# mightypirate1/DRL-Tetris

Hardware: AMD Instinct MI355X
Metric: env-steps/sec at 64k parallel 20x10 boards (higher is better)
Workload: dtype u32

## Files before the change

drl-tetris_amd/csrc/tetris_dev_rollout.h:

```cpp

constexpr int CHAIN_LANES = 64;
constexpr int CHAIN_STREAMS = 3;
template <int P, bool AFFINE, bool FUSED>
__device__ __forceinline__ void chain_body(const KArgs& a) {
    __shared__ __attribute__((aligned(16))) uint32_t s_shapes[SHAPE_WORDS];
    const int lane = threadIdx.x;
    if (a.steps < 0) { chain_census(a, lane == 0); return; }
    constexpr int CMEM = AFFINE ? MEM_AFFINE : MEM_AGENT;
    int wave = blockIdx.x;
    uint32_t xcc = 0;
    const auto report_xcc = [&]() { if (AFFINE && blockIdx.x == 0 && lane == 0) st_flag(a.status + F_XCC0 + (a.xcd_slot & 3u), 0x100u | xcc); };
    if (AFFINE) {
        asm volatile("s_getreg_b32 %0, hwreg(HW_REG_XCC_ID)" : "=s"(xcc));
        xcc &= 0xFu;
        if (xcc != ((a.xcd_base + blockIdx.x) & 7u)) {
            if (lane == 0) st_flag(a.status + F_PLACE, 1u);
            report_xcc();
            return;
        }
        wave = (int)((blockIdx.x & ~7u) | xcc);
        if (wave * CHAIN_LANES >= a.n) { report_xcc(); return; }
    }
    const int i = wave * CHAIN_LANES + lane;
    const bool active = lane < CHAIN_LANES && i < a.n;
    LaneCounters cnt = {0, 0, 0, 0};
    const uint32_t shape_word = d_shape_table.s[lane];
    Game<P> g;
    if (active) policy_draw(a, (uint32_t)i, a.first_step, g.draw0, g.draw1);
    const uint32_t d0 = g.draw0, d1 = g.draw1;
    int stride = a.n_stride;
    asm volatile("" : "+s"(stride));
    RowTable<NWORDS> rows = {};
    RowTable<NGWORDS> grows = {};
    if (!FUSED) {
        TE_UNROLL
        for (int w = 0; w < NWORDS; w++)
            if (P > 1 || (w < NWORDS_HOT && w != W_INCOMING && w != W_HOLE_DRAWS)) {
                uint32_t bytes = (uint32_t)(w * P) * (uint32_t)stride * 4u;
                asm volatile("" : "+s"(bytes));
                rows.bytes[w] = bytes;
            }
        TE_UNROLL
        for (int w = 0; w < NGWORDS; w++) {
            uint32_t bytes = (uint32_t)w * (uint32_t)stride * 4u;
// ... 4 lines not shown
    const uint32_t seen = chain_poll(a, (uint32_t)wave);
    if (seen == a.epoch - 1u) {
        Geo geo = geo_of(a);
        geo.stride = (size_t)stride;
        if (active) {
            if (FUSED) load_game<P>(geo, (size_t)i, g, false, P > 1, true, CMEM);
            else load_game_rows<P>(geo, (size_t)i, rows, grows, g, false, P > 1, true, CMEM);
            g.draw0 = d0; g.draw1 = d1;
        }
        s_shapes[lane] = shape_word;
        __builtin_amdgcn_wave_barrier();
        if (FUSED) {
            if (active) game_run<P, M_ROLLOUT, false, CMEM>(a, i, s_shapes, g, cnt);
        } else if (active) {
            const Ctx cx = make_ctx(a, s_shapes, false, P > 1);
            rollout_step<P>(cx, a, (size_t)i, a.first_step, g, cnt);
            store_game_rows<P>(geo, (size_t)i, rows, grows, g, false, P > 1, true, CMEM);
            report_status(a, g.status);
        }
        asm volatile("s_waitcnt vmcnt(0)" ::: "memory");
        if (lane == 0) {
            if (AFFINE) st_xcd(a.chain + (size_t)wave * CHAIN_STRIDE, a.epoch);
            else st_agent(a.chain + (size_t)wave * CHAIN_STRIDE, a.epoch);
        }
    } else if (!(seen & CHAIN_ABANDONED)) {
        chain_give_up(a, (uint32_t)wave, lane == 0);
    }
    report_xcc();
}
template <int P>
__global__ __launch_bounds__(64) void k_chain(KArgs a) { chain_body<P, false, false>(a); }
template <int P>
__global__ __launch_bounds__(64) void k_chain_affine(KArgs a) { chain_body<P, true, false>(a); }
template <int P>
__global__ __launch_bounds__(64) void k_chain_fused(KArgs a) { chain_body<P, false, true>(a); }
template <int P>
__global__ __launch_bounds__(64) void k_chain_fused_affine(KArgs a) { chain_body<P, true, true>(a); }
template __global__ void k_chain_affine<1>(KArgs);
// ... 45 lines not shown
    }
    if (active) {
        load_game_words<1>(gr, g, ROLL, MEM);
        load_player(br.s, br.o, br.ws, q, false, true, MEM);
        if (CHAIN) { g.draw0 = pd0; g.draw1 = pd1; }
        else if (ROLL) policy_draw(a, (uint32_t)gi, a.first_step, g.draw0, g.draw1);
        else { g.draw0 = a.rot[gi]; g.draw1 = (uint32_t)a.trans[gi] | ((a.player ? (uint32_t)a.player[gi] : 0u) << 8); }
    }
    s_shapes[lane] = shape_word;
    __builtin_amdgcn_wave_barrier();
    Ctx cx = make_ctx(a, s_shapes, false);
    uint32_t my_lines = 0, my_sent = 0;
    int done = 0, out_reward = 0, out_dead = 0;
    {
        int r = 0, t = 0, acting = 0;
        ResetPrefetch rpf;
        rpf.ok = 0; rpf.seed16 = 0; rpf.word = 0;
        uint32_t sent_start = 0;
        uint32_t wa = 0;
        uint32_t undo_pose = 0, undo_group = 0, undo_draws = 0, undo_cleared = 0;
        bool undo_ran = false;
        Player pre;
        if (active) {
            if (ROLL) {
                r = (int)(g.draw0 & 3u); t = (int)(g.draw1 % 10u); acting = (int)(a.first_step % 2ull);
            } else {
                r = (int)(g.draw0 & 3u); t = (int)(g.draw1 & 0xFFu); acting = (int)(g.draw1 >> 8);
            }
            if (ROLL || AUTO) prefetch_reset(cx, episode_seed(a.game_offset + (uint32_t)gi, g.episode + 1), rpf);
            prefetch_next(cx, q, g.seed16, g.status);
            sent_start = q.lines_sent;
            if (!g.round_over && !q.dead && acting == side) play_rt(cx, q, r, t);
            if (!CHAIN && side == 1) pre = q;
            undo_pose = pose_pack(q);
            undo_group = q.pgroup; undo_draws = q.piece_draws;
            undo_cleared = q.lines_cleared; undo_ran = !g.round_over && !q.dead;
            wa = split_settle(cx, g);
        }
        const uint32_t opp_a = __shfl_xor(wa, 32);
        uint32_t wb0 = 0, wb1 = 0;
        if (active) {
            if (side == 1 && (opp_a & XW_DIED)) {
                if (!CHAIN) {
                    q = pre;
// ... 20 lines not shown
        }
        const uint32_t x1 = __shfl_xor(wb1, 32);
        if (active) {
            const uint32_t opp_b = side == 0 ? x1 : x0;
            const int in = (side == 0 && !(opp_b & XW_DIED)) ? xw_sent(opp_b) : 0;
            g.flags = (uint32_t)side;
            done = split_finish(g, in, (opp_b & XW_DEAD_NOW) != 0, (opp_b & XW_ERR) != 0);
            out_reward = q.reward; out_dead = q.dead;
            if (ROLL) {
                g.steps++;
                if (!q.dead) my_lines += (unsigned)q.reward;
                my_sent += (q.lines_sent - sent_start) & 0xFFFFu;
            }
            if ((ROLL || AUTO) && done) {
                g.episode++;
                reset_split(cx, g, episode_seed(a.game_offset + (uint32_t)gi, g.episode));
            }
        }
    }
    const uint32_t opp_lines = __shfl_xor(my_lines, 32), opp_sent = __shfl_xor(my_sent, 32);
    if (active) {
        store_player(br.s, br.o, br.ws, q, false, true, MEM);
        if (!ROLL) {
            if (a.lines) a.lines[(size_t)side * a.n + gi] = (uint8_t)out_reward;
            if (a.dead) a.dead[(size_t)side * a.n + gi] = (uint8_t)out_dead;
        }
        const uint32_t st = g.status | __shfl_xor(g.status, 32);
        if (side == 0) {
            if (!ROLL && a.done) a.done[gi] = (uint8_t)done;
            g.flags = 0;
            g.add_lines = my_lines + opp_lines;
// ... 79 lines not shown
```

drl-tetris_amd/csrc/tetris_engine.h:

```cpp
#pragma once
#include "tetris_layout.h"
#include "tetris_tables.h"

#if defined(__clang__)
#define TE_UNROLL _Pragma("unroll")
#else
#define TE_UNROLL _Pragma("GCC unroll 8")
#endif

namespace te {

TE_HD int ctz32(uint32_t v) { return __builtin_ctz(v); }
TE_HD int clz32(uint32_t v) { return __builtin_clz(v); }
#if defined(__HIP_DEVICE_COMPILE__)
TE_HD uint32_t ld_stream(const uint32_t* p) { return __builtin_nontemporal_load(p); }
TE_HD void st_stream(uint32_t* p, uint32_t v) { __builtin_nontemporal_store(v, p); }
#else
TE_HD uint32_t ld_stream(const uint32_t* p) { return *p; }
TE_HD void st_stream(uint32_t* p, uint32_t v) { *p = v; }
#endif

#if defined(TE_PATH_COUNTERS) && !defined(__HIPCC__)
enum PathCounter { PC_KICK = 0, PC_KICK_2ND, PC_KICK_3RD, PC_KICK_FAILED, PC_KICK_DOWN, PC_DROP_EXACT, PC_RT_OFF_SPAWN,
                   PC_GARBAGE_ROW, PC_GARBAGE_LIFT2, PC_DEATH_GARBAGE, PC_DEATH_SPAWN, PC_TIMER_LOCK, PC_KEY_KICK, PC_KEY_KICK_FAILED,
// ... 43 lines not shown
struct RowStride { size_t ws; };
template <int N>
struct RowTable { uint32_t bytes[N]; };
TE_HD size_t row_bytes(const RowStride& r, int w) { return (size_t)w * r.ws * 4u; }
template <int N>
TE_HD size_t row_bytes(const RowTable<N>& r, int w) { return r.bytes[w]; }
#if defined(__HIP_DEVICE_COMPILE__)
TE_HD void add_word(uint32_t* p, uint32_t v) { (void)__hip_atomic_fetch_add(p, v, __ATOMIC_RELAXED, __HIP_MEMORY_SCOPE_AGENT); }
#else
TE_HD void add_word(uint32_t* p, uint32_t v) { *p += v; }
#endif
#if defined(__HIP_DEVICE_COMPILE__)
TE_HD uint32_t mul24(uint32_t a, uint32_t b) { return __umul24(a, b); }
#else
TE_HD uint32_t mul24(uint32_t a, uint32_t b) { return a * b; }
#endif
TE_HD int imin(int a, int b) { return a < b ? a : b; }
TE_HD int imax(int a, int b) { return a > b ? a : b; }
TE_HD uint32_t f2u(float f) { union { float f; uint32_t u; } v; v.f = f; return v.u; }
TE_HD float u2f(uint32_t u) { union { float f; uint32_t u; } v; v.u = u; return v.f; }

constexpr uint16_t SHAPE_ROWS[7][4] = {
    {0x2260, 0x0710, 0x3220, 0x4700}, {0x2230, 0x1700, 0x6220, 0x0740}, {0x2640, 0x0630, 0x1320, 0x6300},
    {0x2310, 0x3600, 0x4620, 0x0360}, {0x2222, 0x0f00, 0x4444, 0x00f0}, {0x0720, 0x2320, 0x2700, 0x2620},
    {0x0660, 0x0660, 0x0660, 0x0660},
};
TE_HD int spawn_rot(int kind) { return (int)((0x0977u >> (2 * (kind & 7))) & 3u); }
TE_HD int shape_value(int kind) { return (int)((0x06127534u >> (4 * (kind & 7))) & 15u); }

constexpr uint32_t make_shape(int kind, int rot) {
// ... 60 lines not shown
    int q_overflow;
    int32_t time_ms, drop_delay, drop_time, speedup_time, lock_time;
    int32_t combo_start, combo_time, min_remaining;
    uint32_t combo_remaining;
    float incoming;
    uint32_t piece_draws, hole_draws;
    uint32_t pgroup;
    uint32_t lines_sent, lines_cleared, lines_blocked, max_combo, lines_seen, garbage_cleared;
    int32_t qcount[FIFO_CAP];
    int32_t qdelay[FIFO_CAP];
    int q_loaded;
    Raw8 pf_raw;
    int pf_ok;
};

struct ResetPrefetch { uint32_t seed16; uint64_t word; int ok; };

template <int P>
struct Game {
    Player pl[P];
    uint32_t seed16;
    int round_over, last_winner;
    uint32_t flags;
    uint32_t episode;
    uint32_t steps;
    uint32_t add_lines, add_sent;
    uint32_t status;
    uint32_t draw0, draw1;
};

template <class ROWS>
// ... 249 lines not shown
        uint32_t above = (1u << r) - 1u;
        uint32_t keep = ~((above << 1) | 1u);
        if (cx.tint) {
            uint32_t garbage = 0;
            for (int c = 0; c < NCOL; c++) garbage |= q.col[c] & q.tint[0][c] & q.tint[1][c] & q.tint[2][c];
            if ((garbage >> r) & 1u) q.garbage_cleared = (q.garbage_cleared + 1u) & 0xFFFFu;
            for (int k = 0; k < 3; k++)
                for (int c = 0; c < NCOL; c++) q.tint[k][c] = (q.tint[k][c] & keep) | ((q.tint[k][c] & above) << 1);
        }
        for (int c = 0; c < NCOL; c++) q.col[c] = (q.col[c] & keep) | ((q.col[c] & above) << 1);
        cleared++;
    }
    return cleared;
}

TE_HD uint32_t table_byte(const Ctx& cx, uint32_t seed16, uint32_t draw, uint32_t& status) {
    if (draw + cx.margin >= cx.n_draws) {
        status |= ST_NEED_EXTEND;
        if (draw >= cx.n_draws) { status |= ST_STREAM_EXHAUSTED; draw = cx.n_draws - 1; }
    }
    uint32_t chunk = draw / (uint32_t)CHUNK;
    uint32_t r = draw - mul24(chunk, (uint32_t)CHUNK);
    return cx.table[mul24((chunk << 16) + seed16, (uint32_t)CHUNK) + r];
}

TE_HD Raw8 table_group_raw(const Ctx& cx, uint32_t seed16, uint32_t draw, uint32_t& status) {
    if (draw + 8u + cx.margin >= cx.n_draws) {
        status |= ST_NEED_EXTEND;
        if (draw + 8u > cx.n_draws) { status |= ST_STREAM_EXHAUSTED; draw = cx.n_draws - 8u; }
    }
    uint32_t chunk = draw / (uint32_t)CHUNK;
    uint32_t r = draw - mul24(chunk, (uint32_t)CHUNK);
    const uint8_t* p = cx.table + (mul24((chunk << 16) + seed16, (uint32_t)CHUNK) + r);
    Raw8 v;
#if defined(__HIP_DEVICE_COMPILE__)
    const uint2 w = *reinterpret_cast<const uint2*>(p);
    v.lo = w.x; v.hi = w.y;
#else
    v.lo = 0; v.hi = 0;
    for (int k = 0; k < 4; k++) { v.lo |= (uint32_t)p[k] << (8 * k); v.hi |= (uint32_t)p[4 + k] << (8 * k); }
#endif
    return v;
}
TE_HD uint32_t pack_group(Raw8 v) {
    const uint32_t a = v.lo & 0x0F0F0F0Fu, b = v.hi & 0x0F0F0F0Fu;
    uint32_t lo = (a | (a >> 4)) & 0x00FF00FFu; lo = (lo | (lo >> 8)) & 0x0000FFFFu;
    uint32_t hi = (b | (b >> 4)) & 0x00FF00FFu; hi = (hi | (hi >> 8)) & 0x0000FFFFu;
    return lo | (hi << 16);
// ... 79 lines not shown
TE_HD int combo_expire(const Ctx& cx, Player& q, int32_t t) {
    int32_t left = q.combo_start + q.combo_time - t;
    q.combo_remaining = left < 0 ? 0u : ((uint32_t)left & 0xFFFFu);
    if (t > q.combo_start + q.combo_time && q.combo_count != 0) {
        float duration = 1.f + (float)t / 60000.f * 0.1f;
        double v = cx.combo_pow[q.combo_count] * (double)duration;
        int lines = (int)((uint32_t)(int64_t)v & 0xFFFFu);
        q.combo_count = 0;
        q.line_count = 0;
        return lines;
    }
    return 0;
}


TE_HD bool spawn_next(const Ctx& cx, Player& q, uint32_t seed16, uint32_t& status) {
    q.kind = q.next;
    q.rot = spawn_rot(q.kind);
    q.x = (NCOL - 4) / 2;
    q.y = 0;
    if (q.piece_draws + cx.margin >= cx.n_draws) {
        status |= ST_NEED_EXTEND;
        if (q.piece_draws >= cx.n_draws) status |= ST_STREAM_EXHAUSTED;
    }
    q.next = (int)((q.pgroup >> (4u * (q.piece_draws & 7u))) & 7u);
    q.piece_draws++;
    if ((q.piece_draws & 7u) == 0u) {
        q.pgroup = pack_group(q.pf_ok ? q.pf_raw : table_group_raw(cx, seed16, q.piece_draws, status));
        q.pf_ok = 0;
    }
    uint32_t shape = shape_of(cx, q.kind, q.rot);
    if (!fits_spawn_col(cx, q, shape, 0)) { stamp(cx, q, shape); TE_COUNT(PC_DEATH_SPAWN); return true; }
    return false;
}

TE_HD int score_clears(const Ctx& cx, Player& q, int cleared) {
    q.lines_cleared = (q.lines_cleared + (uint32_t)cleared) & 0xFFFFu;
    if (cleared == 0) { q.combo_time -= 200; return 0; }
    int amount = cx.queue ? q_block(q, cleared - 1, q.time_ms, true) : cleared - 1;
    q.lines_sent = (q.lines_sent + (uint32_t)amount) & 0xFFFFu;
    combo_gain(q, q.time_ms, cleared);
    return amount;
}

TE_HD void lock_piece(const Ctx& cx, Player& q) {
    uint32_t shape = shape_of(cx, q.kind, q.rot);
    q.y += drop_distance(cx, q, shape);
    stamp(cx, q, shape);
    q.drop_time = q.time_ms;
    q.lock_armed = 0;
}

TE_HD int settle(const Ctx& cx, Player& q, uint32_t seed16, uint32_t& status) {
    int sent = score_clears(cx, q, clear_rows(cx, q));
    if (spawn_next(cx, q, seed16, status)) return -1;
    return sent;
}

TE_HD bool soft_drop(const Ctx& cx, Player& q) {
    const uint32_t shape = shape_of(cx, q.kind, q.rot);
    if (q.x == (NCOL - 4) / 2 ? fits_spawn_col(cx, q, shape, q.y + 1) : fits_at(cx, q, shape, q.x, q.y + 1)) {
        q.y++;
        q.drop_time = q.time_ms;
        q.lock_armed = 0;
        return true;
    }
    if (!q.lock_armed) q.lock_time = q.time_ms + 400;
    q.lock_armed = 1;
    return false;
}

TE_HD bool gravity_due(Player& q, int32_t t) {
    if (t - q.speedup_time > 3000) {
        if (q.drop_delay > 200) q.drop_delay -= 10;
        else if (q.drop_delay > 100) q.drop_delay -= 5;
        else if (q.drop_delay > 50) q.drop_delay -= 2;
        else if (q.drop_delay > 10) q.drop_delay -= 1;
        q.speedup_time = t;
    }
    if (t - q.drop_time > q.drop_delay) { q.drop_time = t; return true; }
    return false;
}

TE_HD bool push_garbage(const Ctx& cx, Player& q, uint32_t seed16, uint32_t& status) {
    int hole = (int)(table_byte(cx, seed16, q.hole_draws, status) >> 4);
    q.hole_draws++;
    uint32_t bottom = 1u << (cx.H - 1);
    for (int c = 0; c < NCOL; c++) q.col[c] = (q.col[c] >> 1) | (c == hole ? 0u : bottom);
    if (cx.tint)
        for (int k = 0; k < 3; k++)
            for (int c = 0; c < NCOL; c++) q.tint[k][c] = (q.tint[k][c] >> 1) | (c == hole ? 0u : bottom);
    TE_COUNT(PC_GARBAGE_ROW);
    if (q.y > 0) q.y--;
    if (!fits_at(cx, q, shape_of(cx, q.kind, q.rot), q.x, q.y)) {
        if (q.y > 0) { q.y--; TE_COUNT(PC_GARBAGE_LIFT2); }
        else { TE_COUNT(PC_DEATH_GARBAGE); return true; }
    }
    return false;
}

TE_HD int tick(const Ctx& cx, Player& q, int ms, uint32_t seed16, uint32_t& status) {
    q.time_ms += ms;
    if (gravity_due(q, q.time_ms)) soft_drop(cx, q);
    int sent = 0;
    bool finished = false;
    if (q.lock_armed && q.time_ms > q.lock_time && !soft_drop(cx, q)) {
        TE_COUNT(PC_TIMER_LOCK);
        lock_piece(cx, q);
        sent = settle(cx, q, seed16, status);
        finished = true;
    }
    if (!finished) {
        if (cx.queue) {
            int whole = 0;
            while (q.incoming >= 1.0f) { whole++; q.incoming = q.incoming - 1.f; }
            if (whole) q_add(q, whole, q.time_ms, status);
        }
        sent = combo_expire(cx, q, q.time_ms);
        if (sent) {
            if (cx.queue) sent = q_block(q, sent, q.time_ms, false);
            q.lines_sent = (q.lines_sent + (uint32_t)sent) & 0xFFFFu;
        }
        if (cx.queue && q_release(q, q.time_ms))
            if (push_garbage(cx, q, seed16, status)) sent = -1;
    }
    return sent;
}

TE_HD void restart_player(const Ctx& cx, Player& q, uint32_t seed16, uint32_t& status, const ResetPrefetch* pf = nullptr) {
    for (int c = 0; c < NCOL; c++) q.col[c] = 0;
    if (cx.tint)
        for (int k = 0; k < 3; k++)
            for (int c = 0; c < NCOL; c++) q.tint[k][c] = 0;
    q.qlen = 0; q.q_overflow = 0; q.lines_blocked = 0; q.min_remaining = 1000;
    if (cx.queue)
        for (int i = 0; i < FIFO_CAP; i++) { q.qcount[i] = 0; q.qdelay[i] = 0; }
    q.combo_start = 0; q.combo_time = 0; q.max_combo = 0; q.combo_count = 0; q.line_count = 0;
    q.lines_sent = 0; q.lines_cleared = 0; q.garbage_cleared = 0;
    q.speedup_time = 0; q.drop_delay = 1000; q.drop_time = 0; q.lock_time = 0; q.lock_armed = 0;
    q.time_ms = 0; q.incoming = 0.0f; q.lines_seen = 0; q.dead = 0;
    (void)status;
    const uint64_t word = (pf && pf->ok && pf->seed16 == seed16) ? pf->word : cx.start[seed16];
    const uint32_t j = (uint32_t)word & 0xFFu, b0 = ((uint32_t)word >> 8) & 0xFFu, b1 = ((uint32_t)word >> 16) & 0xFFu;
    q.pgroup = (uint32_t)(word >> 32);
    q.kind = (int)(b0 & 7u);
    q.next = (int)(b1 & 7u);
    q.pf_ok = 0;
    q.rot = spawn_rot(q.kind);
    q.x = (NCOL - 4) / 2; q.y = 0;
    q.piece_draws = j + 2; q.hole_draws = 0;
}

template <int P>
TE_HD void reset_game(const Ctx& cx, Game<P>& g, uint32_t seed16, const ResetPrefetch* pf = nullptr) {
    g.round_over = 0;
    int winner = -1, alive = 0;
    TE_UNROLL
    for (int p = 0; p < P; p++)
        if (!g.pl[p].dead) { alive++; winner = p; }
    g.last_winner = winner;
    if (P == 1) g.last_winner = 0;
    if (alive > 1) g.last_winner = -1;
    g.seed16 = seed16 & 0xFFFFu;
    TE_UNROLL
    for (int p = 0; p < P; p++) restart_player(cx, g.pl[p], g.seed16, g.status, pf);
}

TE_HD void prefetch_reset(const Ctx& cx, uint32_t next_seed16, ResetPrefetch& pf) {
    pf.seed16 = next_seed16 & 0xFFFFu;
    pf.word = cx.start[pf.seed16];
    pf.ok = 1;
}

template <int P>
TE_HD void init_game(const Ctx& cx, Game<P>& g, uint32_t seed16) {
    TE_UNROLL
    for (int p = 0; p < P; p++) {
        Player& q = g.pl[p];
        q.reward = 0; q.inc_count = 0; q.combo_remaining = 0; q.dead = 0; q.next = 0; q.kind = 7; q.rot = 0;
        q.q_loaded = 1;
    }
    g.episode = 0; g.steps = 0; g.add_lines = 0; g.add_sent = 0; g.status = 0; g.flags = 0;
    reset_game(cx, g, seed16);
    g.last_winner = -1;
}


// ... 452 lines not shown
        if (p != sender) g.pl[p].incoming = g.pl[p].incoming + each;
}

template <int P>
TE_HD bool confine_errors(Game<P>& g) {
    int err = 0;
    TE_UNROLL
    for (int p = 0; p < P; p++) {
        if (g.status & ST_STREAM_EXHAUSTED) g.pl[p].q_overflow |= ERR_STREAM;
        err |= g.pl[p].q_overflow;
    }
    return err != 0;
}

template <int P>
TE_HD int finish_game(const Ctx& cx, Game<P>& g, int ms) {
    if (g.round_over) return 1;
    bool stop = false;
    TE_UNROLL
    for (int p = 0; p < P; p++) {
        Player& q = g.pl[p];
        if (!stop && !q.dead) {
            const int sent = settle(cx, q, g.seed16, g.status);
            if (sent == -1) { q.dead = 1; stop = true; }
            else if (sent) share_lines<P>(g, p, sent);
        }
    }
    int alive = 0;
    TE_UNROLL
    for (int p = 0; p < P; p++) {
        Player& q = g.pl[p];
        if (!q.dead) {
            const int sent = tick(cx, q, ms, g.seed16, g.status);
            if (sent == -1) q.dead = 1;
            else {
                if (sent) share_lines<P>(g, p, sent);
                alive++;
                q.reward = (int)((q.lines_cleared - q.lines_seen) & 0xFFu);
                q.lines_seen = q.lines_cleared;
                q.inc_count = cx.queue ? (q_total(q) & 255) : 0;
            }
        }
    }
    if (confine_errors<P>(g)) { g.round_over = 1; return 1; }
    if ((P > 1 && alive < 2) || !alive) { g.round_over = 1; return 1; }
    return 0;
}

// ... 27 lines not shown
    }
    if (g.status & ST_STREAM_EXHAUSTED) q.q_overflow |= ERR_STREAM;
    return w | (q.dead ? XW_DEAD_NOW : 0u) | (q.q_overflow ? XW_ERR : 0u);
}

TE_HD int split_finish(Game<1>& g, int lines_in, bool opp_dead, bool opp_err = false) {
    Player& q = g.pl[0];
    if (g.round_over) return 1;
    if (lines_in > 0) q.incoming = q.incoming + (float)lines_in / 1.0f;
    g.flags = (g.flags & ~SPLIT_OPP_DEAD) | (opp_dead ? SPLIT_OPP_DEAD : 0u);
    int alive = (q.dead ? 0 : 1) + (opp_dead ? 0 : 1);
    if (alive < 2 || q.q_overflow || opp_err) { g.round_over = 1; return 1; }
    return 0;
}

TE_HD void reset_split(const Ctx& cx, Game<1>& g, uint32_t seed16) {
    const int side = (int)(g.flags & SPLIT_SIDE);
    const bool me_alive = !g.pl[0].dead, opp_alive = !(g.flags & SPLIT_OPP_DEAD);
    int winner = -1;
    if (me_alive && !opp_alive) winner = side;
    if (opp_alive && !me_alive) winner = 1 - side;
    reset_game<1>(cx, g, seed16);
    g.last_winner = winner;
    g.flags &= ~SPLIT_OPP_DEAD;
}

TE_HD uint32_t episode_seed(uint32_t game, uint32_t episode) { return (12345u + mul24(7919u, game & 0xFFFFu) + mul24(104729u & 0xFFFFu, episode & 0xFFFFu)) & 0xFFFFu; }

TE_HD void philox4x32_10(uint32_t k0, uint32_t c0, uint32_t c1, uint32_t c2, uint32_t out[4]) {
    uint32_t k1 = 0u, c3 = 0u;
    TE_UNROLL
    for (int r = 0; r < 10; r++) {
        uint64_t p0 = (uint64_t)0xD2511F53u * c0;
        uint64_t p1 = (uint64_t)0xCD9E8D57u * c2;
        uint32_t n0 = (uint32_t)(p1 >> 32) ^ c1 ^ k0;
        uint32_t n1 = (uint32_t)p1;
        uint32_t n2 = (uint32_t)(p0 >> 32) ^ c3 ^ k1;
        uint32_t n3 = (uint32_t)p0;
        c0 = n0; c1 = n1; c2 = n2; c3 = n3;
        k0 += 0x9E3779B9u; k1 += 0xBB67AE85u;
    }
    out[0] = c0; out[1] = c1; out[2] = c2; out[3] = c3;
// ... 4 lines not shown
```

drl-tetris_amd/csrc/tetris_kernels.h:

```cpp
#pragma once
#include "../../include/tetris_hip.h"
#include "tetris_engine.h"

namespace te {

struct KArgs {
    uint32_t* state;
    uint32_t* gstate;
    uint32_t* status;
    const uint8_t* table;
    const uint64_t* start;
    const double* combo_pow;
    uint32_t n_draws, margin;
    int H;
    int n_games;
    int n_stride;
    int n_players;
    int nw;
    int n;
    const int32_t* idx;
    const uint8_t* keys;
    const uint8_t* lens;
    int max_keys;
    const uint8_t* rot;
// ... 164 lines not shown
    uint32_t w[4];
    philox4x32_10(a.policy_seed, a.game_offset + slot, (uint32_t)step, (uint32_t)(step >> 32), w);
    w0 = w[0]; w1 = w[1];
}

template <int P, int MODE, bool TINT = false, int MEM = MEM_STREAM>
TE_HD void game_load(const KArgs& a, int i, Game<P>& g) {
    const size_t slot = a.idx ? (size_t)a.idx[i] : (size_t)i;
    if (MODE != M_INIT && MODE != M_SPLIT_INIT)
        load_game<P>(geo_of(a), slot, g, TINT, P > 1 || MODE == M_SPLIT_RESET, MODE == M_ROLLOUT, MEM);
    if (MODE == M_ROLLOUT) policy_draw(a, (uint32_t)slot, a.first_step, g.draw0, g.draw1);
    if (MODE == M_STEP_RT || MODE == M_STEP_RT_AUTO) { g.draw0 = a.rot[i]; g.draw1 = (uint32_t)a.trans[i] | ((a.player ? (uint32_t)a.player[i] : 0u) << 8); }
}

template <int P>
TE_HD void rollout_step(const Ctx& cx, const KArgs& a, size_t slot, unsigned long long step, Game<P>& g, LaneCounters& cnt) {
    TE_UNROLL
    for (int p = 0; p < P; p++) prefetch_next(cx, g.pl[p], g.seed16, g.status);
    ResetPrefetch rpf;
    prefetch_reset(cx, episode_seed(a.game_offset + (uint32_t)slot, g.episode + 1), rpf);
    int r = (int)(g.draw0 & 3u), t = (int)(g.draw1 % 10u);
    int player = P > 1 ? (int)(step % (unsigned long long)P) : 0;
    uint32_t sent_before = 0;
    TE_UNROLL
    for (int p = 0; p < P; p++) sent_before += g.pl[p].lines_sent;
    make_rt<P>(cx, g, player, r, t);
    int done = finish_game<P>(cx, g, a.ms);
    cnt.steps++;
    g.steps++;
    uint32_t sent_after = 0;
    TE_UNROLL
    for (int p = 0; p < P; p++) {
        sent_after += g.pl[p].lines_sent;
        if (!g.pl[p].dead) { cnt.lines += (unsigned)g.pl[p].reward; g.add_lines += (unsigned)g.pl[p].reward; }
    }
    cnt.sent += (sent_after - sent_before) & 0xFFFFu;
    g.add_sent += (sent_after - sent_before) & 0xFFFFu;
    if (done) {
        cnt.episodes++;
        g.episode++;
        reset_game<P>(cx, g, episode_seed(a.game_offset + (uint32_t)slot, g.episode), &rpf);
    }
}

template <int P, int MODE, bool TINT = false, int MEM = MEM_STREAM>
TE_HD void game_run(const KArgs& a, int i, const uint32_t* shapes, Game<P>& g, LaneCounters& cnt) {
    const size_t slot = a.idx ? (size_t)a.idx[i] : (size_t)i;
    Ctx cx = make_ctx(a, shapes, TINT, P > 1 || MODE == M_SPLIT_INIT || MODE == M_SPLIT_RESET);
    if (MODE == M_INIT) init_game<P>(cx, g, (uint32_t)(a.seeds ? (uint16_t)a.seeds[i] : 0));
    if (MODE == M_SPLIT_INIT) {
        init_game<P>(cx, g, (uint32_t)(a.seeds ? (uint16_t)a.seeds[i] : 0));
        g.flags = SPLIT_ON | (a.steps ? SPLIT_SIDE : 0u);
    } else if (MODE == M_SPLIT_RESET) {
        if (P == 1) reset_split(cx, *reinterpret_cast<Game<1>*>(&g), (uint32_t)(a.seeds ? (uint16_t)a.seeds[i] : 0));
    } else if (MODE == M_RESET) {
        reset_game<P>(cx, g, (uint32_t)(a.seeds ? (uint16_t)a.seeds[i] : 0));
// ... 4 lines not shown
        make_keys<P>(cx, a, i, g);
    } else if (MODE == M_FINISH) {
        TE_UNROLL
        for (int p = 0; p < P; p++) prefetch_next(cx, g.pl[p], g.seed16, g.status);
        int done = finish_game<P>(cx, g, a.ms);
        write_outputs<P>(a, i, g, done);
    } else if (MODE == M_STEP_KEYS) {
        TE_UNROLL
        for (int p = 0; p < P; p++) prefetch_next(cx, g.pl[p], g.seed16, g.status);
        make_keys<P>(cx, a, i, g);
        int done = finish_game<P>(cx, g, a.ms);
        write_outputs<P>(a, i, g, done);
    } else if (MODE == M_STEP_RT || MODE == M_STEP_RT_AUTO) {
        TE_UNROLL
        for (int p = 0; p < P; p++) prefetch_next(cx, g.pl[p], g.seed16, g.status);
        ResetPrefetch rpf;
        rpf.ok = 0; rpf.seed16 = 0; rpf.word = 0;
        if (MODE == M_STEP_RT_AUTO) prefetch_reset(cx, episode_seed(a.game_offset + (uint32_t)slot, g.episode + 1), rpf);
        make_rt<P>(cx, g, (int)(g.draw1 >> 8), (int)(g.draw0 & 3u), (int)(g.draw1 & 0xFFu));
        int done = finish_game<P>(cx, g, a.ms);
        write_outputs<P>(a, i, g, done);
        if (MODE == M_STEP_RT_AUTO && done) {
            g.episode++;
            reset_game<P>(cx, g, episode_seed(a.game_offset + (uint32_t)slot, g.episode), &rpf);
        }
    } else if (MODE == M_ROLLOUT) {
        uint32_t earlier = 0;
        for (int s = 0; s < a.steps; s++) {
            unsigned long long step = a.first_step + (unsigned long long)s;
            rollout_step<P>(cx, a, slot, step, g, cnt);
            if (s + 1 < a.steps) {
                policy_draw(a, (uint32_t)slot, step + 1, g.draw0, g.draw1);
                earlier |= g.status; g.status = 0;
            }
        }
        g.status |= earlier;
    }
    store_game<P>(geo_of(a), slot, g, TINT, P > 1 || MODE == M_SPLIT_INIT || MODE == M_SPLIT_RESET,
                  MODE == M_ROLLOUT || MODE == M_INIT || MODE == M_SPLIT_INIT, MEM);
    report_status(a, g.status);
}

constexpr int UNDO_WORDS = 4;
constexpr uint32_t UNDO_RAN = 1u, UNDO_SIMPLE = 2u;
TE_HD Ref undo_ref(const KArgs& a, int i) { Ref r = {a.shadow, (uint32_t)i * 4u, (size_t)a.n_stride}; return r; }
// ... 401 lines not shown
```

drl-tetris_amd/csrc/tetris_plan.h:

```cpp
#pragma once
#include "tetris_kernels.h"

namespace te {

constexpr int PLAN_LANE_LISTS = 16;
constexpr int PLAN_RAW_MAX = 40 * PLAN_LANE_LISTS;

struct PlanArgs {
    KArgs a;
    const uint8_t* player;
    const int32_t* count;
    const uint8_t* lens;
    const uint8_t* keys;
    const int32_t* choice;
    uint32_t* cols;
    int max_lists, max_keys;
};

TE_HD int plan_slab_lane(int j) { return (j & 3) * 10 + (j >> 2); }

TE_HD bool plan_same_list(const uint8_t* ka, int la, const uint8_t* kb, int lb) {
    if (la != lb) return false;
    for (int j = 0; j < la; j++)
        if (ka[j] != kb[j]) return false;
// ... 122 lines not shown
    }
    TE_UNROLL
    for (int p = 0; p < P; p++)
        for (int col = 0; col < NCOL; col++) pa.cols[(((size_t)k * P + p) * NCOL + col) * n + i] = g.pl[p].col[col];
    report_status(a, g.status & ~(uint32_t)(ST_STREAM_EXHAUSTED | ST_FIFO_OVERFLOW));
}

template <int P, bool TINT, bool AUTO>
TE_HD void plan_step_lane(const PlanArgs& pa, int i, const uint32_t* shapes, bool ) {
    const KArgs& a = pa.a;
    Game<P> g;
    load_game<P>(geo_of(a), (size_t)i, g, TINT, P > 1, false);
    const Ctx cx = make_ctx(a, shapes, TINT, P > 1);
    TE_UNROLL
    for (int p = 0; p < P; p++) prefetch_next(cx, g.pl[p], g.seed16, g.status);
    ResetPrefetch rpf;
    rpf.ok = 0; rpf.seed16 = 0; rpf.word = 0;
    if (AUTO) prefetch_reset(cx, episode_seed(a.game_offset + (uint32_t)i, g.episode + 1), rpf);
    const int player = safe_player(pa.player, i, P);
    const int c = imin(pa.count[i], pa.max_lists);
    int len = 1;
    const uint8_t* kp = nullptr;
    if (c >= 1) kp = plan_list(pa, i, imax(0, imin(pa.choice[i], c - 1)), len);
    plan_make_keys<P>(cx, g, player, kp, len);
    const int done = finish_game<P>(cx, g, a.ms);
    write_outputs<P>(a, i, g, done);
    if (AUTO && done) {
        g.episode++;
        reset_game<P>(cx, g, episode_seed(a.game_offset + (uint32_t)i, g.episode), &rpf);
    }
    store_game<P>(geo_of(a), (size_t)i, g, TINT, P > 1, false);
    report_status(a, g.status);
}

struct PlanDeltaArgs {
    Geo geo;
    int H, n;
    const uint8_t* player;
    const int32_t* count;
    const uint32_t* cols;
    int max_lists;
    float small_fill;
    void* deltas;
    void* sums;
// ... 84 lines not shown
```

drl-tetris_amd/csrc/tetris_policy.h:

```cpp
#pragma once
#include "tetris_kernels.h"

namespace te {

constexpr int POLICY_FEATURES = TETRIS_POLICY_FEATURES;
constexpr int POLICY_CANDIDATES = 40;

struct PolicyArgs {
    KArgs a;
    const uint8_t* player;
    int fixed_player;
    const int16_t* weights;
    int per_game;
    int16_t* features;
    int32_t* scores;
    uint8_t* rot;
    uint8_t* trans;
    int32_t* score;
};

struct PolicyBoard {
    uint32_t col[NCOL];
    int kind, rot, x, y;
    bool can;
// ... 164 lines not shown
    load_game<P>(geo_of(a), (size_t)i, g, TINT, P > 1, ROLL);
    const Ctx cx = make_ctx(a, shapes, TINT, P > 1);
    int w[POLICY_FEATURES];
    if (!FROM_SCORES) policy_weights(pa, i, w);
    const int steps = ROLL ? a.steps : 1;
    uint32_t earlier = 0;
    for (int s = 0; s < steps; s++) {
        if (ROLL) { earlier |= g.status; g.status = 0; }
        const unsigned long long step = a.first_step + (unsigned long long)s;
        const int player = ROLL ? (P > 1 ? (int)(step % (unsigned long long)P) : 0) : safe_player(pa.player, i, P);
        int32_t best;
        const int c = FROM_SCORES ? policy_pick_scores(pa, i, best) : policy_pick_board(cx, policy_board_of<P>(g, player), w, a.H, best);
        if (!ROLL) policy_write_choice(pa, i, c, best);
        TE_UNROLL
        for (int p = 0; p < P; p++) prefetch_next(cx, g.pl[p], g.seed16, g.status);
        ResetPrefetch rpf;
        rpf.ok = 0; rpf.seed16 = 0; rpf.word = 0;
        if (AUTO) prefetch_reset(cx, episode_seed(a.game_offset + (uint32_t)i, g.episode + 1), rpf);
        uint32_t sent_before = 0;
        TE_UNROLL
        for (int p = 0; p < P; p++) sent_before += g.pl[p].lines_sent;
        make_rt<P>(cx, g, player, c / 10, c % 10);
        const int done = finish_game<P>(cx, g, a.ms);
        if (!ROLL) write_outputs<P>(a, i, g, done);
        if (ROLL) {
            g.steps++;
            uint32_t sent_after = 0;
            TE_UNROLL
            for (int p = 0; p < P; p++) {
                sent_after += g.pl[p].lines_sent;
                if (!g.pl[p].dead) g.add_lines += (unsigned)g.pl[p].reward;
            }
            g.add_sent += (sent_after - sent_before) & 0xFFFFu;
        }
        if (AUTO && done) {
            g.episode++;
            reset_game<P>(cx, g, episode_seed(a.game_offset + (uint32_t)i, g.episode), &rpf);
        }
    }
    store_game<P>(geo_of(a), (size_t)i, g, TINT, P > 1, ROLL);
    report_status(a, g.status | earlier);
}

TE_HD void policy_game_totals_lane(const Geo& geo, int i, uint32_t* totals) {
    unsigned long long t[4];
    totals_of_game(geo, i, t);
    for (int k = 0; k < 4; k++) totals[(size_t)k * geo.n_games + i] = (uint32_t)t[k];
}

}
```

Measured before the change: 22.35 billion.

## Strength-reduce table indexing, precompute spawn shapes and seeds, drop reset-prefetch checks

Replaces the divide by CHUNK in table lookups with a multiply-and-shift proven exact by static_assert. The per-game part of the episode seed is hoisted out of the step loop. Spawn shapes are computed up front and passed into settle, tick and lock paths, and gravity_due is made branchless. The reset prefetch is used unconditionally, which removes the ok/seed checks and the recomputed start-table load, and the chain epoch-store address is hoisted. Together these aim to cut ALU work, divergence and redundant loads per env step, at the cost of more live registers.

```diff
diff --git a/drl-tetris_amd/csrc/tetris_dev_rollout.h b/drl-tetris_amd/csrc/tetris_dev_rollout.h
--- a/drl-tetris_amd/csrc/tetris_dev_rollout.h
+++ b/drl-tetris_amd/csrc/tetris_dev_rollout.h
@@ -28,6 +28,13 @@
     Game<P> g;
     if (active) policy_draw(a, (uint32_t)i, a.first_step, g.draw0, g.draw1);
     const uint32_t d0 = g.draw0, d1 = g.draw1;
+    uint32_t seed_share = 0;
+    if (!FUSED) {
+        seed_share = seed_of_game(a.game_offset + (uint32_t)i);
+        asm volatile("" : "+v"(seed_share));
+    }
+    uint32_t* epoch_word = a.chain + (size_t)wave * CHAIN_STRIDE;
+    asm volatile("" : "+s"(epoch_word));
     int stride = a.n_stride;
     asm volatile("" : "+s"(stride));
     RowTable<NWORDS> rows = {};
@@ -62,14 +69,18 @@
             if (active) game_run<P, M_ROLLOUT, false, CMEM>(a, i, s_shapes, g, cnt);
         } else if (active) {
             const Ctx cx = make_ctx(a, s_shapes, false, P > 1);
-            rollout_step<P>(cx, a, (size_t)i, a.first_step, g, cnt);
+            rollout_step<P>(cx, a, seed_share, a.first_step, g, cnt);
             store_game_rows<P>(geo, (size_t)i, rows, grows, g, false, P > 1, true, CMEM);
             report_status(a, g.status);
         }
+        uint32_t epoch = a.epoch, no_offset = 0;
+        uint32_t* word = epoch_word;
+        if (AFFINE) asm volatile("" : "+v"(epoch), "+v"(no_offset));
+        else asm volatile("" : "+v"(epoch), "+v"(word));
         asm volatile("s_waitcnt vmcnt(0)" ::: "memory");
         if (lane == 0) {
-            if (AFFINE) st_xcd(a.chain + (size_t)wave * CHAIN_STRIDE, a.epoch);
-            else st_agent(a.chain + (size_t)wave * CHAIN_STRIDE, a.epoch);
+            if (AFFINE) st_xcd((uint32_t*)((char*)word + no_offset), epoch);
+            else st_agent(word, epoch);
         }
     } else if (!(seen & CHAIN_ABANDONED)) {
         chain_give_up(a, (uint32_t)wave, lane == 0);
@@ -145,8 +156,7 @@
     int done = 0, out_reward = 0, out_dead = 0;
     {
         int r = 0, t = 0, acting = 0;
-        ResetPrefetch rpf;
-        rpf.ok = 0; rpf.seed16 = 0; rpf.word = 0;
+        ResetPrefetch rpf = {0u, 0ull};
         uint32_t sent_start = 0;
         uint32_t wa = 0;
         uint32_t undo_pose = 0, undo_group = 0, undo_draws = 0, undo_cleared = 0;
@@ -158,7 +168,7 @@
             } else {
                 r = (int)(g.draw0 & 3u); t = (int)(g.draw1 & 0xFFu); acting = (int)(g.draw1 >> 8);
             }
-            if (ROLL || AUTO) prefetch_reset(cx, episode_seed(a.game_offset + (uint32_t)gi, g.episode + 1), rpf);
+            if (ROLL || AUTO) rpf = prefetch_reset(cx, episode_seed(a.game_offset + (uint32_t)gi, g.episode + 1));
             prefetch_next(cx, q, g.seed16, g.status);
             sent_start = q.lines_sent;
             if (!g.round_over && !q.dead && acting == side) play_rt(cx, q, r, t);
@@ -209,7 +219,7 @@
             }
             if ((ROLL || AUTO) && done) {
                 g.episode++;
-                reset_split(cx, g, episode_seed(a.game_offset + (uint32_t)gi, g.episode));
+                reset_split(cx, g, rpf);
             }
         }
     }
diff --git a/drl-tetris_amd/csrc/tetris_engine.h b/drl-tetris_amd/csrc/tetris_engine.h
--- a/drl-tetris_amd/csrc/tetris_engine.h
+++ b/drl-tetris_amd/csrc/tetris_engine.h
@@ -81,6 +81,12 @@
 TE_HD uint32_t mul24(uint32_t a, uint32_t b) { return __umul24(a, b); }
 #else
 TE_HD uint32_t mul24(uint32_t a, uint32_t b) { return a * b; }
+#endif
+constexpr uint32_t mul24_value(uint32_t a, uint32_t b) { return (a & 0xFFFFFFu) * (b & 0xFFFFFFu); }
+#if defined(__HIP_DEVICE_COMPILE__)
+TE_HD uint32_t pinned(uint32_t v) { asm("" : "+v"(v)); return v; }
+#else
+TE_HD uint32_t pinned(uint32_t v) { return v; }
 #endif
 TE_HD int imin(int a, int b) { return a < b ? a : b; }
 TE_HD int imax(int a, int b) { return a > b ? a : b; }
@@ -171,7 +177,7 @@
     int pf_ok;
 };
 
-struct ResetPrefetch { uint32_t seed16; uint64_t word; int ok; };
+struct ResetPrefetch { uint32_t seed16; uint64_t word; };
 
 template <int P>
 struct Game {
@@ -451,14 +457,34 @@
     return cleared;
 }
 
+constexpr uint32_t CHUNK_MUL = 13444u, CHUNK_SHIFT = 20u;
+constexpr uint32_t chunk_value(uint32_t draw) { return mul24_value(draw >> 3, CHUNK_MUL) >> CHUNK_SHIFT; }
+constexpr uint32_t table_index_value(uint32_t seed16, uint32_t draw) {
+    return mul24_value((chunk_value(draw) << 16) - chunk_value(draw) + seed16, (uint32_t)CHUNK) + draw;
+}
+constexpr bool table_index_is_exact() {
+    for (uint32_t d8 = 0; d8 <= (uint32_t)(MAX_CHUNKS * CHUNK); d8 += 8)
+        for (uint32_t k = 0; k < 8; k += 7)
+            for (uint32_t seed16 = 0; seed16 <= 0xFFFFu; seed16 += 0xFFFFu) {
+                const uint32_t draw = d8 + k;
+                const uint64_t chunk = draw / (uint32_t)CHUNK, want = (chunk * 65536u + seed16) * (uint64_t)CHUNK + (draw - chunk * (uint32_t)CHUNK);
+                if ((((uint64_t)(draw >> 3) * CHUNK_MUL) >> 32) || chunk_value(draw) != chunk) return false;
+                if (((chunk * 65535u + seed16) >> 24) || (want >> 32) || table_index_value(seed16, draw) != want) return false;
+            }
+    return true;
+}
+static_assert(CHUNK % 8 == 0 && table_index_is_exact(), "table_index: the multiply-and-shift forms differ from draw / 624 within the tables");
+TE_HD uint32_t table_index(uint32_t seed16, uint32_t draw) {
+    const uint32_t chunk = mul24(draw >> 3, CHUNK_MUL) >> CHUNK_SHIFT;
+    return pinned(mul24((chunk << 16) - chunk + seed16, (uint32_t)CHUNK) + draw);
+}
+
 TE_HD uint32_t table_byte(const Ctx& cx, uint32_t seed16, uint32_t draw, uint32_t& status) {
     if (draw + cx.margin >= cx.n_draws) {
         status |= ST_NEED_EXTEND;
         if (draw >= cx.n_draws) { status |= ST_STREAM_EXHAUSTED; draw = cx.n_draws - 1; }
     }
-    uint32_t chunk = draw / (uint32_t)CHUNK;
-    uint32_t r = draw - mul24(chunk, (uint32_t)CHUNK);
-    return cx.table[mul24((chunk << 16) + seed16, (uint32_t)CHUNK) + r];
+    return cx.table[table_index(seed16, draw)];
 }
 
 TE_HD Raw8 table_group_raw(const Ctx& cx, uint32_t seed16, uint32_t draw, uint32_t& status) {
@@ -466,9 +492,7 @@
         status |= ST_NEED_EXTEND;
         if (draw + 8u > cx.n_draws) { status |= ST_STREAM_EXHAUSTED; draw = cx.n_draws - 8u; }
     }
-    uint32_t chunk = draw / (uint32_t)CHUNK;
-    uint32_t r = draw - mul24(chunk, (uint32_t)CHUNK);
-    const uint8_t* p = cx.table + (mul24((chunk << 16) + seed16, (uint32_t)CHUNK) + r);
+    const uint8_t* p = cx.table + table_index(seed16, draw);
     Raw8 v;
 #if defined(__HIP_DEVICE_COMPILE__)
     const uint2 w = *reinterpret_cast<const uint2*>(p);
@@ -578,7 +602,9 @@
 }
 
 
-TE_HD bool spawn_next(const Ctx& cx, Player& q, uint32_t seed16, uint32_t& status) {
+TE_HD uint32_t spawn_shape_of(const Ctx& cx, const Player& q) { return shape_of(cx, q.next, spawn_rot(q.next)); }
+
+TE_HD bool spawn_next(const Ctx& cx, Player& q, uint32_t seed16, uint32_t& status, uint32_t shape) {
     q.kind = q.next;
     q.rot = spawn_rot(q.kind);
     q.x = (NCOL - 4) / 2;
@@ -588,15 +614,16 @@
         if (q.piece_draws >= cx.n_draws) status |= ST_STREAM_EXHAUSTED;
     }
     q.next = (int)((q.pgroup >> (4u * (q.piece_draws & 7u))) & 7u);
+    const bool crosses = (q.piece_draws & 7u) == 7u;
     q.piece_draws++;
-    if ((q.piece_draws & 7u) == 0u) {
+    if (crosses) {
         q.pgroup = pack_group(q.pf_ok ? q.pf_raw : table_group_raw(cx, seed16, q.piece_draws, status));
         q.pf_ok = 0;
     }
-    uint32_t shape = shape_of(cx, q.kind, q.rot);
     if (!fits_spawn_col(cx, q, shape, 0)) { stamp(cx, q, shape); TE_COUNT(PC_DEATH_SPAWN); return true; }
     return false;
 }
+TE_HD bool spawn_next(const Ctx& cx, Player& q, uint32_t seed16, uint32_t& status) { return spawn_next(cx, q, seed16, status, spawn_shape_of(cx, q)); }
 
 TE_HD int score_clears(const Ctx& cx, Player& q, int cleared) {
     q.lines_cleared = (q.lines_cleared + (uint32_t)cleared) & 0xFFFFu;
@@ -607,22 +634,22 @@
     return amount;
 }
 
-TE_HD void lock_piece(const Ctx& cx, Player& q) {
-    uint32_t shape = shape_of(cx, q.kind, q.rot);
+TE_HD void lock_piece(const Ctx& cx, Player& q, uint32_t shape) {
     q.y += drop_distance(cx, q, shape);
     stamp(cx, q, shape);
     q.drop_time = q.time_ms;
     q.lock_armed = 0;
 }
-
-TE_HD int settle(const Ctx& cx, Player& q, uint32_t seed16, uint32_t& status) {
+TE_HD void lock_piece(const Ctx& cx, Player& q) { lock_piece(cx, q, shape_of(cx, q.kind, q.rot)); }
+
+TE_HD int settle(const Ctx& cx, Player& q, uint32_t seed16, uint32_t& status, uint32_t spawn_shape) {
     int sent = score_clears(cx, q, clear_rows(cx, q));
-    if (spawn_next(cx, q, seed16, status)) return -1;
+    if (spawn_next(cx, q, seed16, status, spawn_shape)) return -1;
     return sent;
 }
-
-TE_HD bool soft_drop(const Ctx& cx, Player& q) {
-    const uint32_t shape = shape_of(cx, q.kind, q.rot);
+TE_HD int settle(const Ctx& cx, Player& q, uint32_t seed16, uint32_t& status) { return settle(cx, q, seed16, status, spawn_shape_of(cx, q)); }
+
+TE_HD bool soft_drop(const Ctx& cx, Player& q, uint32_t shape) {
     if (q.x == (NCOL - 4) / 2 ? fits_spawn_col(cx, q, shape, q.y + 1) : fits_at(cx, q, shape, q.x, q.y + 1)) {
         q.y++;
         q.drop_time = q.time_ms;
@@ -633,17 +660,17 @@
     q.lock_armed = 1;
     return false;
 }
+TE_HD bool soft_drop(const Ctx& cx, Player& q) { return soft_drop(cx, q, shape_of(cx, q.kind, q.rot)); }
 
 TE_HD bool gravity_due(Player& q, int32_t t) {
-    if (t - q.speedup_time > 3000) {
-        if (q.drop_delay > 200) q.drop_delay -= 10;
-        else if (q.drop_delay > 100) q.drop_delay -= 5;
-        else if (q.drop_delay > 50) q.drop_delay -= 2;
-        else if (q.drop_delay > 10) q.drop_delay -= 1;
-        q.speedup_time = t;
-    }
-    if (t - q.drop_time > q.drop_delay) { q.drop_time = t; return true; }
-    return false;
+    const bool speedup = t - q.speedup_time > 3000;
+    const int32_t d = q.drop_delay;
+    const int32_t less = d > 200 ? 10 : (d > 100 ? 5 : (d > 50 ? 2 : (d > 10 ? 1 : 0)));
+    q.drop_delay = speedup ? d - less : d;
+    q.speedup_time = speedup ? t : q.speedup_time;
+    const bool due = t - q.drop_time > q.drop_delay;
+    q.drop_time = due ? t : q.drop_time;
+    return due;
 }
 
 TE_HD bool push_garbage(const Ctx& cx, Player& q, uint32_t seed16, uint32_t& status) {
@@ -663,14 +690,14 @@
     return false;
 }
 
-TE_HD int tick(const Ctx& cx, Player& q, int ms, uint32_t seed16, uint32_t& status) {
+TE_HD int tick(const Ctx& cx, Player& q, int ms, uint32_t seed16, uint32_t& status, uint32_t shape) {
     q.time_ms += ms;
-    if (gravity_due(q, q.time_ms)) soft_drop(cx, q);
+    if (gravity_due(q, q.time_ms)) soft_drop(cx, q, shape);
     int sent = 0;
     bool finished = false;
-    if (q.lock_armed && q.time_ms > q.lock_time && !soft_drop(cx, q)) {
+    if (q.lock_armed && q.time_ms > q.lock_time && !soft_drop(cx, q, shape)) {
         TE_COUNT(PC_TIMER_LOCK);
-        lock_piece(cx, q);
+        lock_piece(cx, q, shape);
         sent = settle(cx, q, seed16, status);
         finished = true;
     }
@@ -690,8 +717,16 @@
     }
     return sent;
 }
-
-TE_HD void restart_player(const Ctx& cx, Player& q, uint32_t seed16, uint32_t& status, const ResetPrefetch* pf = nullptr) {
+TE_HD int tick(const Ctx& cx, Player& q, int ms, uint32_t seed16, uint32_t& status) { return tick(cx, q, ms, seed16, status, shape_of(cx, q.kind, q.rot)); }
+
+TE_HD ResetPrefetch prefetch_reset(const Ctx& cx, uint32_t next_seed16) {
+    ResetPrefetch pf;
+    pf.seed16 = next_seed16 & 0xFFFFu;
+    pf.word = cx.start[pf.seed16];
+    return pf;
+}
+
+TE_HD void restart_player(const Ctx& cx, Player& q, uint64_t word) {
     for (int c = 0; c < NCOL; c++) q.col[c] = 0;
     if (cx.tint)
         for (int k = 0; k < 3; k++)
@@ -703,8 +738,6 @@
     q.lines_sent = 0; q.lines_cleared = 0; q.garbage_cleared = 0;
     q.speedup_time = 0; q.drop_delay = 1000; q.drop_time = 0; q.lock_time = 0; q.lock_armed = 0;
     q.time_ms = 0; q.incoming = 0.0f; q.lines_seen = 0; q.dead = 0;
-    (void)status;
-    const uint64_t word = (pf && pf->ok && pf->seed16 == seed16) ? pf->word : cx.start[seed16];
     const uint32_t j = (uint32_t)word & 0xFFu, b0 = ((uint32_t)word >> 8) & 0xFFu, b1 = ((uint32_t)word >> 16) & 0xFFu;
     q.pgroup = (uint32_t)(word >> 32);
     q.kind = (int)(b0 & 7u);
@@ -716,7 +749,7 @@
 }
 
 template <int P>
-TE_HD void reset_game(const Ctx& cx, Game<P>& g, uint32_t seed16, const ResetPrefetch* pf = nullptr) {
+TE_HD void reset_game(const Ctx& cx, Game<P>& g, const ResetPrefetch& pf) {
     g.round_over = 0;
     int winner = -1, alive = 0;
     TE_UNROLL
@@ -725,16 +758,12 @@
     g.last_winner = winner;
     if (P == 1) g.last_winner = 0;
     if (alive > 1) g.last_winner = -1;
-    g.seed16 = seed16 & 0xFFFFu;
+    g.seed16 = pf.seed16;
     TE_UNROLL
-    for (int p = 0; p < P; p++) restart_player(cx, g.pl[p], g.seed16, g.status, pf);
-}
-
-TE_HD void prefetch_reset(const Ctx& cx, uint32_t next_seed16, ResetPrefetch& pf) {
-    pf.seed16 = next_seed16 & 0xFFFFu;
-    pf.word = cx.start[pf.seed16];
-    pf.ok = 1;
-}
+    for (int p = 0; p < P; p++) restart_player(cx, g.pl[p], pf.word);
+}
+template <int P>
+TE_HD void reset_game(const Ctx& cx, Game<P>& g, uint32_t seed16) { reset_game<P>(cx, g, prefetch_reset(cx, seed16)); }
 
 template <int P>
 TE_HD void init_game(const Ctx& cx, Game<P>& g, uint32_t seed16) {
@@ -1217,14 +1246,14 @@
 }
 
 template <int P>
-TE_HD int finish_game(const Ctx& cx, Game<P>& g, int ms) {
+TE_HD int finish_game(const Ctx& cx, Game<P>& g, int ms, const uint32_t* spawn_shapes = nullptr) {
     if (g.round_over) return 1;
     bool stop = false;
     TE_UNROLL
     for (int p = 0; p < P; p++) {
         Player& q = g.pl[p];
         if (!stop && !q.dead) {
-            const int sent = settle(cx, q, g.seed16, g.status);
+            const int sent = spawn_shapes ? settle(cx, q, g.seed16, g.status, spawn_shapes[p]) : settle(cx, q, g.seed16, g.status);
             if (sent == -1) { q.dead = 1; stop = true; }
             else if (sent) share_lines<P>(g, p, sent);
         }
@@ -1234,7 +1263,7 @@
     for (int p = 0; p < P; p++) {
         Player& q = g.pl[p];
         if (!q.dead) {
-            const int sent = tick(cx, q, ms, g.seed16, g.status);
+            const int sent = (P == 1 && spawn_shapes) ? tick(cx, q, ms, g.seed16, g.status, spawn_shapes[0]) : tick(cx, q, ms, g.seed16, g.status);
             if (sent == -1) q.dead = 1;
             else {
                 if (sent) share_lines<P>(g, p, sent);
@@ -1292,18 +1321,33 @@
     return 0;
 }
 
-TE_HD void reset_split(const Ctx& cx, Game<1>& g, uint32_t seed16) {
+TE_HD void reset_split(const Ctx& cx, Game<1>& g, const ResetPrefetch& pf) {
     const int side = (int)(g.flags & SPLIT_SIDE);
     const bool me_alive = !g.pl[0].dead, opp_alive = !(g.flags & SPLIT_OPP_DEAD);
     int winner = -1;
     if (me_alive && !opp_alive) winner = side;
     if (opp_alive && !me_alive) winner = 1 - side;
-    reset_game<1>(cx, g, seed16);
+    reset_game<1>(cx, g, pf);
     g.last_winner = winner;
     g.flags &= ~SPLIT_OPP_DEAD;
 }
-
-TE_HD uint32_t episode_seed(uint32_t game, uint32_t episode) { return (12345u + mul24(7919u, game & 0xFFFFu) + mul24(104729u & 0xFFFFu, episode & 0xFFFFu)) & 0xFFFFu; }
+TE_HD void reset_split(const Ctx& cx, Game<1>& g, uint32_t seed16) { reset_split(cx, g, prefetch_reset(cx, seed16)); }
+
+constexpr uint32_t SEED_BASE = 12345u, SEED_PER_GAME = 7919u, SEED_PER_EPISODE = 104729u;
+constexpr uint32_t episode_seed_value(uint32_t game, uint32_t episode) {
+    return (SEED_BASE + mul24_value(SEED_PER_GAME, game & 0xFFFFu) + mul24_value(SEED_PER_EPISODE & 0xFFFFu, episode & 0xFFFFu)) & 0xFFFFu;
+}
+constexpr bool episode_seed_is_exact() {
+    constexpr uint32_t edge[] = {0u, 1u, 0x7FFFu, 0x8000u, 0xFFFEu, 0xFFFFu, 0x10000u, 0x10001u, 0x7FFFFFFFu, 0x80000000u, 0xFFFEFFFFu, 0xFFFF0000u, 0xFFFFFFFEu, 0xFFFFFFFFu};
+    for (uint32_t game : edge)
+        for (uint32_t episode : edge)
+            if (episode_seed_value(game, episode) != ((SEED_BASE + SEED_PER_GAME * game + SEED_PER_EPISODE * episode) & 0xFFFFu)) return false;
+    return true;
+}
+static_assert(episode_seed_is_exact(), "episode_seed: the masked 24-bit form differs from the 32-bit arithmetic");
+TE_HD uint32_t seed_of_game(uint32_t game) { return SEED_BASE + pinned(mul24(SEED_PER_GAME, game & 0xFFFFu)); }
+TE_HD uint32_t episode_seed_from(uint32_t game_share, uint32_t episode) { return (game_share + pinned(mul24(SEED_PER_EPISODE & 0xFFFFu, episode & 0xFFFFu))) & 0xFFFFu; }
+TE_HD uint32_t episode_seed(uint32_t game, uint32_t episode) { return episode_seed_from(seed_of_game(game), episode); }
 
 TE_HD void philox4x32_10(uint32_t k0, uint32_t c0, uint32_t c1, uint32_t c2, uint32_t out[4]) {
     uint32_t k1 = 0u, c3 = 0u;
diff --git a/drl-tetris_amd/csrc/tetris_kernels.h b/drl-tetris_amd/csrc/tetris_kernels.h
--- a/drl-tetris_amd/csrc/tetris_kernels.h
+++ b/drl-tetris_amd/csrc/tetris_kernels.h
@@ -202,18 +202,21 @@
 }
 
 template <int P>
-TE_HD void rollout_step(const Ctx& cx, const KArgs& a, size_t slot, unsigned long long step, Game<P>& g, LaneCounters& cnt) {
+TE_HD void rollout_step(const Ctx& cx, const KArgs& a, uint32_t seed_share, unsigned long long step, Game<P>& g, LaneCounters& cnt) {
+    uint32_t spawn_shapes[P];
     TE_UNROLL
-    for (int p = 0; p < P; p++) prefetch_next(cx, g.pl[p], g.seed16, g.status);
-    ResetPrefetch rpf;
-    prefetch_reset(cx, episode_seed(a.game_offset + (uint32_t)slot, g.episode + 1), rpf);
+    for (int p = 0; p < P; p++) {
+        prefetch_next(cx, g.pl[p], g.seed16, g.status);
+        spawn_shapes[p] = spawn_shape_of(cx, g.pl[p]);
+    }
+    const ResetPrefetch rpf = prefetch_reset(cx, episode_seed_from(seed_share, g.episode + 1));
     int r = (int)(g.draw0 & 3u), t = (int)(g.draw1 % 10u);
     int player = P > 1 ? (int)(step % (unsigned long long)P) : 0;
     uint32_t sent_before = 0;
     TE_UNROLL
     for (int p = 0; p < P; p++) sent_before += g.pl[p].lines_sent;
     make_rt<P>(cx, g, player, r, t);
-    int done = finish_game<P>(cx, g, a.ms);
+    int done = finish_game<P>(cx, g, a.ms, spawn_shapes);
     cnt.steps++;
     g.steps++;
     uint32_t sent_after = 0;
@@ -227,7 +230,7 @@
     if (done) {
         cnt.episodes++;
         g.episode++;
-        reset_game<P>(cx, g, episode_seed(a.game_offset + (uint32_t)slot, g.episode), &rpf);
+        reset_game<P>(cx, g, rpf);
     }
 }
 
@@ -262,21 +265,21 @@
     } else if (MODE == M_STEP_RT || MODE == M_STEP_RT_AUTO) {
         TE_UNROLL
         for (int p = 0; p < P; p++) prefetch_next(cx, g.pl[p], g.seed16, g.status);
-        ResetPrefetch rpf;
-        rpf.ok = 0; rpf.seed16 = 0; rpf.word = 0;
-        if (MODE == M_STEP_RT_AUTO) prefetch_reset(cx, episode_seed(a.game_offset + (uint32_t)slot, g.episode + 1), rpf);
+        ResetPrefetch rpf = {0u, 0ull};
+        if (MODE == M_STEP_RT_AUTO) rpf = prefetch_reset(cx, episode_seed(a.game_offset + (uint32_t)slot, g.episode + 1));
         make_rt<P>(cx, g, (int)(g.draw1 >> 8), (int)(g.draw0 & 3u), (int)(g.draw1 & 0xFFu));
         int done = finish_game<P>(cx, g, a.ms);
         write_outputs<P>(a, i, g, done);
         if (MODE == M_STEP_RT_AUTO && done) {
             g.episode++;
-            reset_game<P>(cx, g, episode_seed(a.game_offset + (uint32_t)slot, g.episode), &rpf);
+            reset_game<P>(cx, g, rpf);
         }
     } else if (MODE == M_ROLLOUT) {
         uint32_t earlier = 0;
+        const uint32_t seed_share = seed_of_game(a.game_offset + (uint32_t)slot);
         for (int s = 0; s < a.steps; s++) {
             unsigned long long step = a.first_step + (unsigned long long)s;
-            rollout_step<P>(cx, a, slot, step, g, cnt);
+            rollout_step<P>(cx, a, seed_share, step, g, cnt);
             if (s + 1 < a.steps) {
                 policy_draw(a, (uint32_t)slot, step + 1, g.draw0, g.draw1);
                 earlier |= g.status; g.status = 0;
diff --git a/drl-tetris_amd/csrc/tetris_plan.h b/drl-tetris_amd/csrc/tetris_plan.h
--- a/drl-tetris_amd/csrc/tetris_plan.h
+++ b/drl-tetris_amd/csrc/tetris_plan.h
@@ -160,9 +160,8 @@
     const Ctx cx = make_ctx(a, shapes, TINT, P > 1);
     TE_UNROLL
     for (int p = 0; p < P; p++) prefetch_next(cx, g.pl[p], g.seed16, g.status);
-    ResetPrefetch rpf;
-    rpf.ok = 0; rpf.seed16 = 0; rpf.word = 0;
-    if (AUTO) prefetch_reset(cx, episode_seed(a.game_offset + (uint32_t)i, g.episode + 1), rpf);
+    ResetPrefetch rpf = {0u, 0ull};
+    if (AUTO) rpf = prefetch_reset(cx, episode_seed(a.game_offset + (uint32_t)i, g.episode + 1));
     const int player = safe_player(pa.player, i, P);
     const int c = imin(pa.count[i], pa.max_lists);
     int len = 1;
@@ -173,7 +172,7 @@
     write_outputs<P>(a, i, g, done);
     if (AUTO && done) {
         g.episode++;
-        reset_game<P>(cx, g, episode_seed(a.game_offset + (uint32_t)i, g.episode), &rpf);
+        reset_game<P>(cx, g, rpf);
     }
     store_game<P>(geo_of(a), (size_t)i, g, TINT, P > 1, false);
     report_status(a, g.status);
diff --git a/drl-tetris_amd/csrc/tetris_policy.h b/drl-tetris_amd/csrc/tetris_policy.h
--- a/drl-tetris_amd/csrc/tetris_policy.h
+++ b/drl-tetris_amd/csrc/tetris_policy.h
@@ -202,9 +202,8 @@
         if (!ROLL) policy_write_choice(pa, i, c, best);
         TE_UNROLL
         for (int p = 0; p < P; p++) prefetch_next(cx, g.pl[p], g.seed16, g.status);
-        ResetPrefetch rpf;
-        rpf.ok = 0; rpf.seed16 = 0; rpf.word = 0;
-        if (AUTO) prefetch_reset(cx, episode_seed(a.game_offset + (uint32_t)i, g.episode + 1), rpf);
+        ResetPrefetch rpf = {0u, 0ull};
+        if (AUTO) rpf = prefetch_reset(cx, episode_seed(a.game_offset + (uint32_t)i, g.episode + 1));
         uint32_t sent_before = 0;
         TE_UNROLL
         for (int p = 0; p < P; p++) sent_before += g.pl[p].lines_sent;
@@ -223,7 +222,7 @@
         }
         if (AUTO && done) {
             g.episode++;
-            reset_game<P>(cx, g, episode_seed(a.game_offset + (uint32_t)i, g.episode), &rpf);
+            reset_game<P>(cx, g, rpf);
         }
     }
     store_game<P>(geo_of(a), (size_t)i, g, TINT, P > 1, ROLL);
```

After: 23.04 billion, median of 6. 1.03x the previous value.
